# jakubbober/discrete-curvature-rewiring

Hardware: AMD Instinct MI355X
Metric: SDRF iterations/sec (higher is better)
Workload: dtype f64; 1 GPU; S100k: preferential-attachment graph N=100000 m=10 E=999900 (PCG64 seed 12345), Balanced Forman curvature, full recompute every iteration, remove_edges=True, tau=163.0, removal_bound=0.95; parallelism=single GPU

## Files before the change

### discrete-curvature-rewiring_amd/csrc/dcr_bfc_h2.hip

```cpp
#include <algorithm>
#include <climits>
#include <cstdio>
#include <cstdlib>
#include <cstring>
#include <vector>

#include "dcr_bfc_common.h"

namespace dcr {

constexpr unsigned H2_EMPTY = 0xFFFFFFFFu;
constexpr unsigned H2_NBR = 0x80000000u;
constexpr int H2_CLASSES = 5;
constexpr int H2_WB = 4;
__device__ inline unsigned h2_rec_t(int T, int deg) { return (unsigned)T | ((unsigned)deg << 16); }
static_assert(H2_MAXDEG < 65536, "record packing");
constexpr int H2_SMALL_DEG = 64;
#ifndef H2_Q
#define H2_Q 2
#endif
#ifndef H2_QL
#define H2_QL 2
#endif
constexpr int H2_QCAP = 128;
// ... 993 lines not shown
    int pln = sc->pln;
#pragma unroll 1
    while (true) {
        const int i = lcur + lane;
        const unsigned item = i < ls.n ? ls.items[i] : 0xFFFFFFFFu;
        const bool mine = i < ls.n && (int)(item >> 19) == bidx;
        const int cnt = __popcll(__ballot(mine));
        if (cnt == 0) break;
        const int s = (int)(item & 0x1FFFu), r = (int)((item >> 13) & 63u);
        const unsigned w = mine ? t.key[s] : 0u;
        h2_settle<L1, EXS>(t, sc, mine, mine ? s : -1, r, w, pln, tk, al, tbase);
        lcur += cnt;
        if (cnt < 64) break;
    }
    if (lane == 0) sc->pln = pln;
    h2_wave_sync();
}

__device__ inline void h2_batch_begin(const H2Tasks tk, H2Alloc &al, H2Scratch *sc, int k, int &tbase, int &trow, int rev = -1) {
    const int lane = threadIdx.x & 63;
    const unsigned long long below = (1ull << lane) - 1ull;
    sc->rowT[lane] = 0;
    sc->rowPos[lane] = 0;
    sc->rowMx[lane] = 0;
    sc->rowRev[lane] = rev;
    if (lane == 0) sc->pln = 0;
    int dummy_c, dummy_p;
    const unsigned long long rows = __ballot(k >= 0);
    if (!h2_pool_reserve(tk, al, __popcll(rows), 0, 0, tbase, dummy_c, dummy_p)) tbase = -1;
    trow = __popcll(rows & below);
    sc->trank[lane] = (unsigned char)trow;
    trow += tbase;
}

template <int L1, int EXS, bool PARTS>
__device__ inline void h2_batch_end(const View &g, const H2Tasks tk, H2Alloc &al, int u, int2 ru, int i, int k, int2 rk, int tbase,
                                    int trow, int part, const H2Tab t, H2Scratch *sc, uint4 *rec, const unsigned *items = nullptr,
                                    int ifrom = 0, int ito = 0) {
    const int lane = threadIdx.x & 63;
    int T = sc->rowT[lane], pos = sc->rowPos[lane], mx = sc->rowMx[lane];
    const int rev = sc->rowRev[lane];
    bool listed = tbase >= 0 && k >= 0 && T > 0 && pos > 0 && rev >= 0 && rev < g.cap_total;
    int ep;
    const int Pn = h2_prefix(listed ? T : 0, ep);
    int p0 = 0;
    if (Pn > 0) {
        int dummy_t, dummy_c;
        if (!h2_pool_reserve(tk, al, 0, 0, Pn, dummy_t, dummy_c, p0)) listed = false;
    }
    if (__ballot(listed) != 0ull) {
        const int pln = sc->pln;
        if (pln <= H2_PLCAP) {
            sc->poff[lane] = listed ? p0 + ep : -1;
            h2_wave_sync();
            for (int j = lane; j < pln; j += 64) {
                const int r = sc->plr[j];
                if (sc->poff[r] >= 0) tk.part[atomicAdd(&sc->poff[r], 1)] = (int32_t)sc->plt[j];
            }
            h2_wave_sync();
        } else if (items) {
            sc->poff[lane] = listed ? p0 + ep : -1;
            h2_wave_sync();
            for (int j = ifrom + lane; j < ito; j += 64) {
                const unsigned item = items[j];
                const int s2 = (int)(item & 0x1FFFu), r = (int)((item >> 13) & 63u);
                if ((h2_cnt_get(t.cnt, s2) & 0x8000u) && sc->poff[r] >= 0) tk.part[atomicAdd(&sc->poff[r], 1)] = (int32_t)t.key[s2];
            }
            h2_wave_sync();
        } else {
            const bool shortrow = listed && rk.y <= H2_SHORT_ROW;
            if (shortrow) h2_partners_short<L1, EXS>(g, tk, u, rk, p0 + ep, T, t);
            unsigned long long todo = __ballot(listed && !shortrow);
            while (todo) {
                const int l = __ffsll((long long)todo) - 1;
                todo &= todo - 1;
                const int2 rv = make_int2(__shfl(rk.x, l), __shfl(rk.y, l));
                h2_partners_of_row<L1, EXS>(g, tk, u, rv, __shfl(p0 + ep, l), __shfl(T, l), t);
            }
        }
    }
    if (tbase >= 0 && k >= 0) {
        tk.task[trow] = listed ? make_uint4((unsigned)(ru.x + i), (unsigned)(p0 + ep), (unsigned)T, (unsigned)u | tk.retry_flag)
                               : make_uint4(0u, 0u, H2_TASK_VOID, 0u);
    }
    if (listed) {
        pos = 0;
        mx = 0;
    }
    if (k >= 0) {
        const int64_t slot = (int64_t)ru.x + i;
        if (rev < 0 || rev >= g.cap_total) {
            row_ok(g, make_int2(-1, rev), 33, u, k);
        } else if (!PARTS) {
            rec[slot] = make_uint4((unsigned)pos, (unsigned)mx, h2_rec_t(T, ru.y), (unsigned)rev);
        } else {
            unsigned *r4 = reinterpret_cast<unsigned *>(rec + slot);
            if (pos) atomicAdd(&r4[0], (unsigned)pos);
            if (mx) atomicMax(&r4[1], (unsigned)mx);
            if (part == 0) {
                r4[2] = h2_rec_t(T, ru.y);
                r4[3] = (unsigned)rev;
            }
        }
    }
}

constexpr int H2_JOIN_MAXM = 256;
__device__ inline int h2_probe_partners(const H2EdgeSet es, int w, const int32_t *pt, int np);

template <int L1, int EXS, int NW>
__device__ inline bool h2_join_prepare(const View &g, const H2Tab t, int2 ru, const H2List &ls) {
    constexpr int NT = 64 * NW, PER = EXS / NT;
    static_assert(PER >= 2 && PER % 2 == 0, "a thread owns whole cursor words");
    static_assert(EXS / 2 <= (1 << L1) / 32, "the cursors fit B1");
    static_assert(NW * H2_ITEMS < 65536 && EXS <= 8192, "16-bit cursors, 13-bit slots");
    const int tid = (int)threadIdx.x, lane = tid & 63, wid = tid >> 6;
    unsigned *cur = t.b1;
    int n[PER], sum = 0, most = 0;
#pragma unroll
    for (int q = 0; q < PER; ++q) {
        const unsigned c16 = h2_cnt_get(t.cnt, tid * PER + q);
        n[q] = ((c16 & 0x8000u) || c16 < 2u) ? 0 : (int)c16;
        sum += n[q];
        most = n[q] > most ? n[q] : most;
    }
    if (__syncthreads_or(most > H2_JOIN_MAXM)) return false;
    int excl;
    const int wtot = h2_prefix(sum, excl);
    if (lane == 0) t.wsum[wid] = wtot;
    __syncthreads();
    int off = excl;
    for (int w = 0; w < wid; ++w) off += t.wsum[w];
#pragma unroll
    for (int q = 0; q < PER; q += 2) {
        const unsigned lo = (unsigned)off;
        off += n[q];
        const unsigned hi = (unsigned)off;
        off += n[q + 1];
        cur[(tid * PER + q) >> 1] = lo | (hi << 16);
    }
    __syncthreads();
    for (int base = 0; base < ls.n; base += 64) {
        const int j = base + lane;
        if (j >= ls.n) continue;
        const unsigned item = ls.items[j];
        const int s = (int)(item & 0x1FFFu), r = (int)((item >> 13) & 63u), b = (int)(item >> 19);
        const unsigned c16 = h2_cnt_get(t.cnt, s);
        if ((c16 & 0x8000u) || c16 < 2u) continue;
        const int row = (b * 64 + r) * NW + wid;
        if (row >= ru.y) {
            row_ok(g, make_int2(-1, row), 44, ru.y, (int)item);
            continue;
        }
        const int v = g.col[ru.x + row];
        const unsigned old = atomicAdd(&cur[s >> 1], 1u << ((s & 1) * 16));
        const int p = (int)((old >> ((s & 1) * 16)) & 0xFFFFu);
        if (p < NW * H2_ITEMS) ls.srt[p] = v;
        else row_ok(g, make_int2(-1, p), 45, s, (int)c16);
    }
    __syncthreads();
    return true;
}

template <int L1, int EXS, int NW, bool PARTS>
__device__ inline void h2_batch_join(const View &g, const H2Tasks tk, H2Alloc &al, int u, int2 ru, int i, int k, int2 rk, int part,
                                     const H2Tab t, H2Scratch *sc, uint4 *rec, const H2List &ls, int &lcur, int bidx, int rev) {
    const int lane = threadIdx.x & 63;
    sc->rowT[lane] = 0;
    sc->rowPos[lane] = 0;
    sc->rowMx[lane] = 0;
    sc->rowRev[lane] = rev;
    if (lane == 0) sc->pln = 0;
    h2_wave_sync();
    const int lfrom = lcur;
#pragma unroll 1
    while (true) {
        const int j = lcur + lane;
        const unsigned item = j < ls.n ? ls.items[j] : 0xFFFFFFFFu;
        const bool mine = j < ls.n && (int)(item >> 19) == bidx;
        const int cnt = __popcll(__ballot(mine));
        if (cnt == 0) break;
        if (mine && (h2_cnt_get(t.cnt, (int)(item & 0x1FFFu)) & 0x8000u)) atomicAdd(&sc->rowT[(item >> 13) & 63u], 1);
        lcur += cnt;
        if (cnt < 64) break;
    }
    h2_wave_sync();
    const unsigned *cur = t.b1;
#pragma unroll 1
    for (int base = lfrom; base < lcur; base += 64) {
        const int j = base + lane;
        const bool have = j < lcur;
        const unsigned item = have ? ls.items[j] : 0u;
        const int s = (int)(item & 0x1FFFu), r = (int)((item >> 13) & 63u);
        const int vr = __shfl(k, r);
        if (!have) continue;
        const unsigned c16 = h2_cnt_get(t.cnt, s);
        if (c16 & 0x8000u) continue;
        const int m = (int)(c16 & 0x7FFFu);
        int c = m - 1;
        if (c <= 0) continue;
        if (sc->rowT[r] > 0 && vr >= 0) {
            const int end = (int)((cur[s >> 1] >> ((s & 1) * 16)) & 0xFFFFu);
            if (end >= m && end <= NW * H2_ITEMS) {
                c -= h2_probe_partners(tk.es, vr, ls.srt + (end - m), m);
            } else {
                row_ok(g, make_int2(-1, end), 46, s, m);
                c = 0;
            }
        }
        if (c > 0) {
            atomicAdd(&sc->rowPos[r], 1);
            atomicMax(&sc->rowMx[r], c);
        }
    }
    h2_wave_sync();
    h2_batch_end<L1, EXS, PARTS>(g, tk, al, u, ru, i, k, rk, -1, 0, part, t, sc, rec);
}

template <int L1, int EXS, int NW, bool PARTS, int PHASE>
__device__ inline void h2_stream(const View &g, const H2Tasks tk, H2Alloc &al, int u, int2 ru, int part, int nparts,
                                 const H2Tab t, H2Scratch *sc, uint4 *rec, int k0, int2 rk0, H2List &ls) {
    const int lane = threadIdx.x & 63;
    const int wid = (int)(threadIdx.x >> 6);
    int qn = 0;
    int lcur = 0;
    if (PHASE == 0 && ru.y > 64 * NW * H2_REV_BATCHES) ls.over = true;
    for (int base = 0; base < ru.y; base += 64 * NW) {
        const int i = base + lane * NW + wid;
        int k = k0;
        int2 rk = rk0;
        if (base > 0) {
            k = -1;
            rk = make_int2(0, 0);
            if (i < ru.y) {
                k = g.col[ru.x + i];
                if (k >= 0 && k < g.n && k != u) {
                    rk = g.rowinfo[k];
                    if (!row_ok(g, rk, 32, k, u)) rk = make_int2(0, 0);
                } else {
                    k = -1;
                }
            }
        }
        const int np = rk.y > 0 ? ((rk.x + rk.y + 3) >> 2) - (rk.x >> 2) : 0;
        int poff_lane;
        const int P = h2_prefix(np, poff_lane);
        if (P == 0) continue;
        const int bidx = base / (64 * NW);
        int tbase = -1, trow = 0;
        if (PHASE == 2 && !ls.over) {
            if (ls.join) {
                h2_batch_join<L1, EXS, NW, PARTS>(g, tk, al, u, ru, i, k, rk, part, t, sc, rec, ls, lcur, bidx, ls.revs[bidx * 64 + lane]);
                h2_wave_sync();
                continue;
            }
            h2_batch_begin(tk, al, sc, k, tbase, trow, ls.revs[bidx * 64 + lane]);
            h2_wave_sync();
            const int lfrom = lcur;
            h2_settle_items<L1, EXS>(t, sc, ls, lcur, bidx, tk, al, tbase);
            h2_batch_end<L1, EXS, PARTS>(g, tk, al, u, ru, i, k, rk, tbase, trow, part, t, sc, rec, ls.items, lfrom, lcur);
            h2_wave_sync();
            continue;
        }
        if (PHASE == 0 && !ls.over) ls.revs[bidx * 64 + lane] = -1;
        sc->desc[lane] = rk;
        sc->poff[lane] = poff_lane;
        if (lane == 0) sc->poff[64] = P;
        if (PHASE == 2) h2_batch_begin(tk, al, sc, k, tbase, trow);
        h2_wave_sync();
        const bool listing = PHASE == 1 && !ls.over;
        auto flags = [&](const int4 w, unsigned vm, int r, int a) -> unsigned {
            const unsigned kk[4] = {(unsigned)w.x, (unsigned)w.y, (unsigned)w.z, (unsigned)w.w};
            const unsigned isu = h2_eq4(kk, (unsigned)u) & vm;
            if (PHASE == 2 && isu) sc->rowRev[r] = a + __ffs((int)isu) - 1;
            if (listing && isu) ls.revs[bidx * 64 + r] = a + __ffs((int)isu) - 1;
            unsigned valid = vm & ~isu;
            if (PARTS && PHASE != 2 && !listing) {
#pragma unroll
                for (int jj = 0; jj < 4; ++jj)
                    if (h2_part(kk[jj], nparts) != part) valid &= ~(1u << jj);
            }
            if (PHASE == 0) {
                h2_mark4<L1>(t.b1, t.b2, kk, valid);
                return 0u;
            }
            return h2_again4<L1>(t.b2, kk, valid);
        };
        h2_for_pieces_queued<(PARTS ? H2_QL : H2_Q)>(g.col, sc->desc, sc->poff, poff_lane, P, qn, flags,
                             [&](int idx, unsigned key, int r) {
                                 sc->qw[idx] = key;
                                 if (PHASE != 0) sc->qr[idx] = (unsigned char)r;
                                 if (PHASE == 1) sc->qb[idx] = (unsigned char)bidx;
                             },
                             [&]() { h2_drain<L1, EXS, PHASE, PARTS>(t, sc, qn, tk, al, tbase, ls, part, nparts); });
        if (PHASE == 2) {
            h2_drain<L1, EXS, PHASE, PARTS>(t, sc, qn, tk, al, tbase, ls, part, nparts);
            h2_batch_end<L1, EXS, PARTS>(g, tk, al, u, ru, i, k, rk, tbase, trow, part, t, sc, rec);
        }
        h2_wave_sync();
    }
    if (qn > 0) h2_drain<L1, EXS, PHASE, PARTS>(t, sc, qn, tk, al, -1, ls, part, nparts);
}

constexpr int H2_NPB = 12;
template <int L1, int EXS, int NW, bool PARTS>
__device__ inline bool h2_node_fast(const View &g, const H2Tasks tk, H2Alloc &al, int u, int2 ru, int part, int nparts,
                                    const H2Tab t, H2Scratch *sc, uint4 *rec, bool &ok, H2List &ls) {
    const int tid = (int)threadIdx.x, lane = tid & 63, wid = tid >> 6;
    constexpr int NT = 64 * NW, NP = H2_NPB;
    const unsigned long long below = (1ull << lane) - 1ull;
    if (ru.y > 64 * NW) return false;
    const int i = lane * NW + wid;
    int k = -1;
    int2 rk = make_int2(0, 0);
    if (i < ru.y) {
        k = g.col[ru.x + i];
        if (k >= 0 && k < g.n && k != u) {
            rk = g.rowinfo[k];
            if (!row_ok(g, rk, 32, k, u)) rk = make_int2(0, 0);
        } else {
            k = -1;
        }
    }
    const int np = rk.y > 0 ? ((rk.x + rk.y + 3) >> 2) - (rk.x >> 2) : 0;
    int poff_lane;
    const int P = h2_prefix(np, poff_lane);
    if (__syncthreads_or(P > 64 * NP)) return false;
    {
        uint4 *z = reinterpret_cast<uint4 *>(t.b1);
        constexpr int NZ = ((1 << L1) / 32 + (1 << (L1 - 2)) / 32) / 4;
        for (int j = tid; j < NZ; j += NT) z[j] = make_uint4(0u, 0u, 0u, 0u);
        uint4 *k4 = reinterpret_cast<uint4 *>(t.key);
        for (int j = tid; j < EXS / 4; j += NT) k4[j] = make_uint4(H2_EMPTY, H2_EMPTY, H2_EMPTY, H2_EMPTY);
        uint4 *c4 = reinterpret_cast<uint4 *>(t.cnt);
        for (int j = tid; j < EXS / 8; j += NT) c4[j] = make_uint4(0u, 0u, 0u, 0u);
        if (tid == 0) *t.full = 0;
    }
    sc->desc[lane] = rk;
    sc->poff[lane] = poff_lane;
    if (lane == 0) sc->poff[64] = P;
    h2_wave_sync();
    int4 w[NP];
    unsigned long long meta[NP];
#pragma unroll
    for (int q = 0; q < NP; ++q) {
        const int j = 64 * q + lane;
        w[q] = make_int4(0, 0, 0, 0);
        meta[q] = 0ull;
        const int jf = 64 * q, jl = jf + 63 < P ? jf + 63 : P - 1;
        if (jf >= P) continue;
        const int r = h2_piece_row(sc->poff, poff_lane, j < P ? j : jl, jf, jl);
        if (j < P) {
            const int2 d = sc->desc[r];
            const int a = (d.x & ~3) + 4 * (j - sc->poff[r]);
            w[q] = load_piece(g.col, a);
            meta[q] = (unsigned long long)h2_piece_mask(a, d.x, d.x + d.y) | ((unsigned long long)r << 8) | ((unsigned long long)(unsigned)a << 16);
        }
    }
    __syncthreads();
    if (k >= 0) {
        const int sl = h2_insert<EXS>(t.key, (unsigned)k);
        if (sl < 0) *t.full = 1;
        else h2_cnt_flag(t.cnt, sl);
        h2_seed<L1>(t.b1, t.b2, (unsigned)k);
    }
    __syncthreads();
#pragma unroll
    for (int q = 0; q < NP; ++q) {
        if (64 * q >= P) continue;
        const unsigned kk[4] = {(unsigned)w[q].x, (unsigned)w[q].y, (unsigned)w[q].z, (unsigned)w[q].w};
        unsigned valid = (unsigned)meta[q] & 0xFu & ~h2_eq4(kk, (unsigned)u);
        if (PARTS) {
#pragma unroll
            for (int jj = 0; jj < 4; ++jj)
                if (h2_part(kk[jj], nparts) != part) valid &= ~(1u << jj);
        }
        meta[q] |= (unsigned long long)valid << 4;
        h2_mark4<L1>(t.b1, t.b2, kk, valid);
    }
    __syncthreads();
    int qn = 0, tbase = -1, trow = 0;
    sc->rowRev[lane] = -1;
    h2_wave_sync();
    {
        unsigned fl[NP];
#pragma unroll
        for (int q = 0; q < NP; ++q) {
            fl[q] = 0u;
            if (64 * q >= P) continue;
            const unsigned kk[4] = {(unsigned)w[q].x, (unsigned)w[q].y, (unsigned)w[q].z, (unsigned)w[q].w};
            const unsigned valid = (unsigned)(meta[q] >> 4) & 0xFu;
            const unsigned isu = h2_eq4(kk, (unsigned)u) & (unsigned)meta[q] & 0xFu;
            if (isu) sc->rowRev[(int)((meta[q] >> 8) & 0xFFull)] = (int)(meta[q] >> 16) + __ffs((int)isu) - 1;
            fl[q] = h2_again4<L1>(t.b2, kk, valid);
        }
#pragma unroll 1
        while (true) {
            bool stop = false;
#pragma unroll
            for (int q = 0; q < NP; ++q) {
                if (64 * q >= P) continue;
                const unsigned kk[4] = {(unsigned)w[q].x, (unsigned)w[q].y, (unsigned)w[q].z, (unsigned)w[q].w};
#pragma unroll
                for (int jj = 0; jj < 4; ++jj) {
                    const bool p = (fl[q] >> jj) & 1u;
                    const unsigned long long m = __ballot(p);
                    if (m == 0ull) continue;
                    if (stop || qn + __popcll(m) > H2_QCAP) {
                        stop = true;
                        continue;
                    }
                    if (p) {
                        const int idx = qn + __popcll(m & below);
                        sc->qw[idx] = kk[jj];
                        sc->qr[idx] = (unsigned char)((meta[q] >> 8) & 0xFFull);
                        sc->qb[idx] = 0;
                        fl[q] &= ~(1u << jj);
                    }
                    qn += __popcll(m);
                }
            }
            if (qn > 0) h2_drain<L1, EXS, 1, PARTS>(t, sc, qn, tk, al, -1, ls, part, nparts);
            if (!stop) break;
        }
    }
    __syncthreads();
    ok = *t.full == 0;
    ls.join = !__syncthreads_or(ls.over) && ok;
    if (ls.join) ls.join = h2_join_prepare<L1, EXS, NW>(g, t, ru, ls);
    if (ls.join) {
        int lcur = 0;
        const int myrev = sc->rowRev[lane];
        h2_wave_sync();
        h2_batch_join<L1, EXS, NW, PARTS>(g, tk, al, u, ru, i, k, rk, part, t, sc, rec, ls, lcur, 0, myrev);
    } else if (ok) {
        if (tid == 0) atomicAdd(&tk.res->h2_fallback, 1);
        if (!ls.over) {
            int lcur = 0;
            const int myrev = sc->rowRev[lane];
            h2_wave_sync();
            h2_batch_begin(tk, al, sc, k, tbase, trow, myrev);
            h2_wave_sync();
            h2_settle_items<L1, EXS>(t, sc, ls, lcur, 0, tk, al, tbase);
            h2_batch_end<L1, EXS, PARTS>(g, tk, al, u, ru, i, k, rk, tbase, trow, part, t, sc, rec, ls.items, 0, lcur);
        } else {
            h2_stream<L1, EXS, NW, PARTS, 2>(g, tk, al, u, ru, part, nparts, t, sc, rec, k, rk, ls);
        }
    }
    __syncthreads();
    return true;
}

template <int L1, int EXS, int NW, bool PARTS>
__device__ inline bool h2_node(const View &g, const H2Tasks tk, H2Alloc &al, int u, int2 ru, int part, int nparts,
                               const H2Tab t, H2Scratch *sc, uint4 *rec, H2List &ls) {
    const int tid = (int)threadIdx.x;
    constexpr int NT = 64 * NW;
    if constexpr (!PARTS) {
        bool ok_fast = true;
        if (h2_node_fast<L1, EXS, NW, PARTS>(g, tk, al, u, ru, part, nparts, t, sc, rec, ok_fast, ls)) return ok_fast;
    }
    int k0 = -1;
    int2 rk0 = make_int2(0, 0);
    {
        const int i0 = (tid & 63) * NW + (tid >> 6);
        if (i0 < ru.y) {
            k0 = g.col[ru.x + i0];
            if (k0 >= 0 && k0 < g.n && k0 != u) {
                rk0 = g.rowinfo[k0];
                if (!row_ok(g, rk0, 32, k0, u)) rk0 = make_int2(0, 0);
            } else {
                k0 = -1;
            }
        }
    }
    {
        uint4 *z = reinterpret_cast<uint4 *>(t.b1);
        constexpr int NZ = ((1 << L1) / 32 + (1 << (L1 - 2)) / 32) / 4;
        for (int i = tid; i < NZ; i += NT) z[i] = make_uint4(0u, 0u, 0u, 0u);
        uint4 *k4 = reinterpret_cast<uint4 *>(t.key);
        for (int i = tid; i < EXS / 4; i += NT) k4[i] = make_uint4(H2_EMPTY, H2_EMPTY, H2_EMPTY, H2_EMPTY);
        uint4 *c4 = reinterpret_cast<uint4 *>(t.cnt);
        for (int i = tid; i < EXS / 8; i += NT) c4[i] = make_uint4(0u, 0u, 0u, 0u);
        if (tid == 0) *t.full = 0;
    }
    __syncthreads();
    for (int i = tid; i < ru.y; i += NT) {
        const int k = g.col[ru.x + i];
        if (k >= 0 && k < g.n && k != u) {
            const int s = h2_insert<EXS>(t.key, (unsigned)k);
            if (s < 0) *t.full = 1;
            else h2_cnt_flag(t.cnt, s);
            h2_seed<L1>(t.b1, t.b2, (unsigned)k);
        }
    }
    __syncthreads();
    h2_stream<L1, EXS, NW, PARTS, 0>(g, tk, al, u, ru, part, nparts, t, sc, rec, k0, rk0, ls);
    __syncthreads();
    h2_stream<L1, EXS, NW, PARTS, 1>(g, tk, al, u, ru, part, nparts, t, sc, rec, k0, rk0, ls);
    __syncthreads();
    const bool ok = *t.full == 0;
    ls.join = !__syncthreads_or(ls.over) && ok;
    if (ls.join) ls.join = h2_join_prepare<L1, EXS, NW>(g, t, ru, ls);
    if (!ls.join && ok && tid == 0) atomicAdd(&tk.res->h2_fallback, 1);
    if (ok) h2_stream<L1, EXS, NW, PARTS, 2>(g, tk, al, u, ru, part, nparts, t, sc, rec, k0, rk0, ls);
    __syncthreads();
    return ok;
}

template <int L1, int EXS, int NW, bool PARTS>
__global__ void __launch_bounds__(64 * NW) __attribute__((amdgpu_waves_per_eu(3))) k_h2_block(View g, H2Tasks tk, const int4 *units, const int32_t *count, int64_t unit_cap,
                                                       uint4 *rec, H2Retry rt, int is_retry) {
    __shared__ __attribute__((aligned(16))) unsigned bits[(1 << L1) / 32 + (1 << (L1 - 2)) / 32];
    __shared__ __attribute__((aligned(16))) unsigned key[EXS];
    __shared__ __attribute__((aligned(16))) unsigned cnt[EXS / 2];
    __shared__ H2Scratch sc_all[NW];
    __shared__ int full;
    __shared__ int wsum[NW];
    const int wid = threadIdx.x >> 6;
    const int total = *count;
    if (total < 0 || total > unit_cap) {
        row_ok(g, make_int2(-1, total), 37, 0, 0);
        return;
    }
    const H2Tab t{bits, bits + (1 << L1) / 32, key, cnt, &full, wsum};
    H2Alloc al;
    for (int64_t it = blockIdx.x; it < total; it += gridDim.x) {
        const int4 un = units[it];
        const int u = un.x;
        const int nparts = PARTS ? (int)((unsigned)un.y >> 16) : 1, part = PARTS ? (un.y & 0xFFFF) : 0;
        bool ok = u >= 0 && u < g.n && nparts >= 1 && part < nparts;
        int2 ru = make_int2(0, 0);
        if (ok) {
            ru = g.rowinfo[u];
            ok = row_ok(g, ru, 38, u, (int)it) && ru.y > 0 && ru.y <= H2_MAXDEG;
        }
        if (!ok) continue;
        H2List ls = h2_list_of(tk.lists, NW);
        const bool unit_ok = h2_node<L1, EXS, NW, PARTS>(g, tk, al, u, ru, part, nparts, t, &sc_all[wid], rec, ls);
        if (!unit_ok) {
            if (threadIdx.x == 0) {
                if (is_retry) {
                    rt.res->h2_status = 1;
                    atomicAdd(&rt.res->h2_failed[5], 1);
                } else {
                    h2_retry_push(rt, u, ru.y, PARTS ? 4 : 3);
                }
            }
        }
    }
    h2_void_candidates(tk, al.c_cur, al.c_end);
    h2_void_tasks(tk, al.t_cur, al.t_end);
}

__device__ inline int h2_probe_partners(const H2EdgeSet es, int w, const int32_t *pt, int np) {
    int found = 0;
    for (int j = 0; j < np; j += 8) {
        int tt[8];
#pragma unroll
        for (int q = 0; q < 8; ++q) tt[q] = j + q < np ? pt[j + q] : -1;
        unsigned long long key[8], k0[8], h[8];
        unsigned bw[8], bb[8];
#pragma unroll
        for (int q = 0; q < 8; ++q) {
            key[q] = h2_edge_key(w, tt[q] < 0 ? w : tt[q]);
            bb[q] = h2_bloom_bit(key[q], es.bloom_bits);
            bw[q] = es.bloom[bb[q] >> 5];
        }
#pragma unroll
        for (int q = 0; q < 8; ++q) {
            const bool maybe = tt[q] >= 0 && ((bw[q] >> (bb[q] & 31u)) & 1u);
            h[q] = h2_eset_slot(key[q], es.bits);
            k0[q] = maybe ? es.tab[h[q]] : H2_ESET_EMPTY;
        }
#pragma unroll
        for (int q = 0; q < 8; ++q) {
            bool hit = k0[q] == key[q];
            if (!hit && k0[q] != H2_ESET_EMPTY) hit = h2_eset_has(es, w, tt[q]);
            found += hit ? 1 : 0;
        }
    }
    return found;
}

__global__ void __launch_bounds__(256) k_h2_triangles(H2EdgeSet es, H2Tasks tk, uint4 *rec, const int32_t *status, int second) {
    const int cand_now = *tk.n_cand;
    const int first = second ? *tk.n_done : 0;
    const int total = cand_now < tk.cand_cap ? cand_now : (int)tk.cand_cap;
    if (!second && blockIdx.x == 0 && threadIdx.x == 0) *tk.n_done = cand_now;
    if (*status != 0) return;
    if (total <= first || first < 0) return;
    const int lane = threadIdx.x & 63;
    for (int64_t base = first + (((int64_t)blockIdx.x * 256 + threadIdx.x) & ~63ll); base < total; base += (int64_t)gridDim.x * 256) {
        const int64_t i = base + lane;
        int c = 0;
        unsigned slot = 0xFFFFFFFFu;
        if (i < total) {
            const int4 cd = tk.cand[i];
            const uint4 ts = (cd.z >= 0 && cd.z < tk.task_cap) ? tk.task[cd.z] : make_uint4(0u, 0u, H2_TASK_VOID, 0u);
            const bool skip = ts.z == H2_TASK_VOID || (!(ts.w & 0x80000000u) && ((unsigned)tk.weight[ts.w & 0x7FFFFFFFu] & 0x80000000u));
            if (!skip) {
                slot = ts.x;
                c = cd.y - h2_probe_partners(es, cd.x, tk.part + ts.y, (int)ts.z);
            }
        }
        const unsigned prev = (unsigned)__shfl_up((int)slot, 1);
        const bool head = lane == 0 || prev != slot;
        const unsigned long long heads = __ballot(head);
        const int seg = __popcll(heads & ((2ull << lane) - 1ull));
        int n = c > 0 ? 1 : 0, mx = c > 0 ? c : 0;
#pragma unroll
        for (int off = 1; off < 64; off <<= 1) {
            const int s2 = __shfl_up(seg, off), n2 = __shfl_up(n, off), m2 = __shfl_up(mx, off);
            if (lane >= off && s2 == seg) {
                n += n2;
                mx = m2 > mx ? m2 : mx;
            }
        }
        const bool tail = lane == 63 || ((heads >> (lane + 1)) & 1ull);
        if (tail && n > 0 && slot != 0xFFFFFFFFu) {
            unsigned *r4 = reinterpret_cast<unsigned *>(rec + slot);
            atomicAdd(&r4[0], (unsigned)n);
            atomicMax(&r4[1], (unsigned)mx);
        }
    }
}

__global__ void __launch_bounds__(256) k_h2_weight(View g, int32_t *weight) {
    const int64_t s = (int64_t)blockIdx.x * 256 + threadIdx.x;
    const int lane = threadIdx.x & 63;
    int u = -1, val = 0;
    if (s < g.cap_total) {
        const int us = g.slot_row[s];
        const int v = g.col[s];
        const bool uok = us >= 0 && us < g.n, vok = v >= 0 && v < g.n;
        const int2 ru = g.rowinfo[uok ? us : 0];
        const int dv = g.rowinfo[vok ? v : 0].y;
        if (uok) {
            u = us;
            if (vok && s >= ru.x && (int)(s - ru.x) < ru.y) val = dv;
        }
    }
#pragma unroll
    for (int off = 1; off < 64; off <<= 1) {
        const int t = __shfl_up(val, off), uu = __shfl_up(u, off);
        if (lane >= off && uu == u) val += t;
    }
    const int un = __shfl_down(u, 1);
    if (u >= 0 && val > 0 && (lane == 63 || un != u)) atomicAdd(&weight[u], val);
}

constexpr int H2_NB = H2_CLASSES * H2_WB;
__device__ inline void h2_clear_result(DevResult *res, int tid, int half, bool flags_cleared) {
    if (tid == 0 && flags_cleared) res->touched_n = 0;
    if (tid < 8) res->misc[tid] = 0;
    if (tid < H2_NB) {
        res->h2_bucket[half][tid] = 0;
        res->h2_fill[half][tid] = 0;
    }
    if (tid < H2_CLASSES) res->h2_count[tid] = 0;
    if (tid == 0) {
        res->h2_status = 0;
        res->h2_retry = 0;
        for (int p = 0; p < 2; ++p) res->h2_ntask[p] = res->h2_ncand[p] = res->h2_npart[p] = res->h2_ncand_done[p] = 0;
        for (int c = 0; c < 6; ++c) res->h2_failed[c] = 0;
        res->h2_fallback = 0;
        res->flag_too_big = 0;
    }
}
struct H2Lists {
    int4 *units[H2_CLASSES];
    int64_t cap[H2_CLASSES];
};
constexpr int H2_PLAN_THREADS = 1024;

__device__ inline void h2_classify(int d, int S, int &cls, int &wb, int &nparts) {
    nparts = 1;
    int lo = 0;
    if (d <= H2_SMALL_DEG && S <= h2_maxw(2)) {
        cls = S <= h2_maxw(0) ? 0 : S <= h2_maxw(1) ? 1 : 2;
        lo = cls == 0 ? 0 : h2_maxw(cls - 1);
        wb = (int)((int64_t)(S - lo) * H2_WB / (h2_maxw(cls) - lo + 1));
    } else if (S <= h2_maxw(3) && d + S / 4 <= h2_keycap(3)) {
// ... 158 lines not shown
        bool want[Q];
#pragma unroll
        for (int q = 0; q < Q; ++q) {
            const int64_t s = s0 + q * stride;
            const bool in = s < g.cap_total;
            u[q] = in ? g.slot_row[s] : -1;
            v[q] = in ? g.col[s] : -1;
            a[q] = in ? rec[s] : make_uint4(0u, 0u, 0u, 0u);
        }
        int2 ru[Q];
        int dv[Q], rcol[Q], rrow[Q];
        uint4 b[Q];
        bool rok[Q];
#pragma unroll
        for (int q = 0; q < Q; ++q) {
            want[q] = u[q] >= 0 && u[q] < g.n && v[q] > u[q] && v[q] < g.n;
            const int64_t r = (int64_t)a[q].w;
            rok[q] = want[q] && r >= 0 && r < g.cap_total;
            ru[q] = make_int2(0, 0);
            dv[q] = 0;
            rcol[q] = rrow[q] = -1;
            b[q] = make_uint4(0u, 0u, 0u, 0u);
            if (want[q]) ru[q] = g.rowinfo[u[q]];
            if (rok[q]) {
                b[q] = rec[r];
                dv[q] = (int)(b[q].z >> 16);
                if (s0 + q * stride == 0) {
                    rcol[q] = g.col[r];
                    rrow[q] = g.slot_row[r];
                } else {
                    rcol[q] = (int64_t)b[q].w == s0 + q * stride ? u[q] : -1;
                    rrow[q] = v[q];
                }
            }
        }
#pragma unroll
        for (int q = 0; q < Q; ++q) {
            const int64_t s = s0 + q * stride;
            if (!want[q]) continue;
            if (s < ru[q].x || (int)(s - ru[q].x) >= ru[q].y) continue;
            double val;
            if (ru[q].y == 1 || (rok[q] && dv[q] == 1)) {
                val = 0.0;
            } else {
                if (!rok[q] || rcol[q] != u[q] || rrow[q] != v[q]) {
                    row_ok(g, make_int2(-1, (int)a[q].w), 39, u[q], v[q]);
                    continue;
                }
                if ((a[q].z & 0xFFFFu) != (b[q].z & 0xFFFFu) || (int)(a[q].z >> 16) != ru[q].y) {
                    row_ok(g, make_int2(-1, (int)a[q].z), 40, u[q], v[q]);
                    continue;
                }
                const int gam = (int)(a[q].y > b[q].y ? a[q].y : b[q].y);
                val = bfc_formula(ru[q].y, dv[q], (int)(a[q].z & 0xFFFFu), (int)b[q].x, (int)a[q].x, gam);
            }
            curv[s] = val;
            ext_take(lo_v, lo_s, val, (int)s, 0);
            ext_take(hi_v, hi_s, val, (int)s, 1);
        }
    }
    ext_wave_reduce(lo_v, lo_s, 0);
    ext_wave_reduce(hi_v, hi_s, 1);
    if ((threadIdx.x & 63) == 0) {
        const int w = (int)blockIdx.x * 4 + (int)(threadIdx.x >> 6);
        part_min[w] = ext_make(lo_v, lo_s);
        part_max[w] = ext_make(hi_v, hi_s);
    }
}

bool h2_grow_pools(dcr_graph *g) {
    const DevResult &h = *g->hres.p;
    const int64_t t = std::max(h.h2_ntask[0], h.h2_ntask[1]), c = std::max(h.h2_ncand[0], h.h2_ncand[1]), p = std::max(h.h2_npart[0], h.h2_npart[1]);
    if (h.h2_ntask[0] < 0 || h.h2_ntask[1] < 0 || h.h2_ncand[0] < 0 || h.h2_ncand[1] < 0 || h.h2_npart[0] < 0 || h.h2_npart[1] < 0) return false;
    if (t < 0 || c < 0 || p < 0) return false;
    g->h2_want[0] = std::max<int64_t>(g->h2_want[0], 2 * t + 4096);
    g->h2_want[1] = std::max<int64_t>(g->h2_want[1], 2 * c + 65536);
    g->h2_want[2] = std::max<int64_t>(g->h2_want[2], 2 * p + 65536);
    return true;
}

static int ensure_h2(dcr_graph *g) {
    if (g->h2_weight.cap < g->n + 64) g->h2_weight_valid = false;
    DCR_TRY(g->h2_weight.grow(g->n + 64));
    DCR_TRY(g->h2_rec.grow(g->cap_total + 64));
    int bits = 10;
    while ((1ll << bits) < g->cap_total) ++bits;
    if (g->h2_eset_bits != bits || !g->h2_eset.p) {
        DCR_TRY(g->h2_eset.alloc((int64_t)1 << bits));
        g->h2_eset_bits = bits;
        g->h2_eset_valid = false;
    }
    int bbits = 16;
    while ((1ll << bbits) < 4 * g->cap_total) ++bbits;
    if (g->h2_bloom_bits != bbits || !g->h2_bloom.p) {
        DCR_TRY(g->h2_bloom.alloc(((int64_t)1 << bbits) / 32));
        g->h2_bloom_bits = bbits;
        g->h2_eset_valid = false;
    }
    const int64_t need[H2_CLASSES] = {g->n + 64, g->n + 64, g->n + 64, g->n + 64, g->n + g->cap_total / 4 + 64};
    for (int c = 0; c < H2_CLASSES; ++c) DCR_TRY(g->h2_units[c].grow(need[c]));
    DCR_TRY(g->h2_retry.grow(g->n + g->cap_total / 4 + 64));
    DCR_TRY(g->h2_task.grow(2 * std::max<int64_t>(g->cap_total + 4096, g->h2_want[0])));
    DCR_TRY(g->h2_cand.grow(2 * std::max<int64_t>(2 * g->cap_total + 65536, g->h2_want[1])));
    DCR_TRY(g->h2_part.grow(2 * std::max<int64_t>(g->cap_total + 65536, g->h2_want[2])));
    const int cus = g->num_cu > 0 ? g->num_cu : 256;
    DCR_TRY(g->h2_lists.grow((int64_t)cus * (16 + 12) * H2_LIST_WORDS));
    return DCR_OK;
}

template <int C>
static void launch_h2_small(dcr_graph *g, const View &vw, const H2Retry &rt, hipStream_t st) {
    constexpr int H2_WPB = h2_wpb(C);
    constexpr int NP = h2_maxw(C) / 256 + 1;
    auto kern = k_h2_small<h2_l1(C), h2_exs(C), h2_clcap(C), H2_WPB, NP>;
    static int per_cu_res = 0;
    if (per_cu_res == 0) {
        int nb = 0;
        if (hipOccupancyMaxActiveBlocksPerMultiprocessor(&nb, kern, 64 * H2_WPB, 0) != hipSuccess || nb < 1) {
            (void)hipGetLastError();
            nb = (160 * 1024) / (H2_WPB * (int)sizeof(H2Small<h2_l1(C), h2_exs(C), h2_clcap(C)>));
            if (nb > 32 / H2_WPB) nb = 32 / H2_WPB;
        }
        per_cu_res = nb < 1 ? 1 : nb;
    }
    int64_t grid = (int64_t)g->num_cu * per_cu_res;
    const int64_t units = g->h2_last_count[C] >= 0 ? (int64_t)g->h2_last_count[C] + g->h2_last_count[C] / 32 + 8 : g->n;
    if (grid > (units + H2_WPB - 1) / H2_WPB) grid = (units + H2_WPB - 1) / H2_WPB;
    if (grid < 1) grid = 1;
    hipLaunchKernelGGL(kern, dim3((unsigned)grid), dim3(64 * H2_WPB), 0, st, vw,
                       g->h2_units[C].p, &g->dres.p->h2_count[C], g->h2_units[C].cap, g->h2_rec.p, rt);
}

template <int C, bool PARTS>
static void launch_h2_block(dcr_graph *g, const View &vw, const H2Tasks &tk, const H2Retry &rt, const int4 *units,
                            const int32_t *count, int64_t cap, int64_t units_hint, int is_retry, hipStream_t st) {
    int64_t grid = units_hint;
    const int64_t most = (int64_t)g->num_cu * (C == 3 ? 3 : 1);
    if (grid > most) grid = most;
    if (grid < 1) grid = 1;
    hipLaunchKernelGGL((k_h2_block<h2_l1(C), h2_exs(C), h2_waves(C), PARTS>), dim3((unsigned)grid), dim3(64 * h2_waves(C)), 0,
                       st, vw, tk, units, count, cap, g->h2_rec.p, rt, is_retry);
}

int launch_curvature_pass_h2(dcr_graph *g) {
    if (g->num_cu <= 0) {
        g->num_cu = 256;
        hipDeviceProp_t prop;
        if (hipGetDeviceProperties(&prop, g->device) == hipSuccess && prop.multiProcessorCount > 0)
            g->num_cu = prop.multiProcessorCount;
    }
    DCR_TRY(ensure_h2(g));
    View vw{g->rowinfo.p, g->col.p, g->slot_row.p, g->cap_total, g->dres.p->misc, nullptr, (int32_t)g->n, 0};
    H2Lists L;
    for (int c = 0; c < H2_CLASSES; ++c) {
        L.units[c] = g->h2_units[c].p;
        L.cap[c] = g->h2_units[c].cap;
    }
    int32_t *status = &g->dres.p->h2_status;
    const H2Retry rt{g->h2_retry.p, g->h2_retry.cap, g->h2_weight.p, g->dres.p};
    const int64_t tcap = g->h2_task.cap / 2, ccap = g->h2_cand.cap / 2, pcap = g->h2_part.cap / 2;
    DevResult *dr = g->dres.p;
    unsigned *lists_L = g->h2_lists.p, *lists_M = g->h2_lists.p + (int64_t)g->num_cu * 16 * H2_LIST_WORDS;
    const H2EdgeSet es{g->h2_eset.p, g->h2_eset_bits, g->h2_bloom.p, g->h2_bloom_bits};
    H2Tasks tk{g->h2_task.p, g->h2_cand.p, g->h2_part.p, tcap, ccap, pcap, &dr->h2_ntask[0], &dr->h2_ncand[0], &dr->h2_npart[0],
               &dr->h2_ncand_done[0], g->dres.p, g->h2_weight.p, 0u, lists_L, es};
    const H2Tasks tkM{g->h2_task.p + tcap, g->h2_cand.p + ccap, g->h2_part.p + pcap, tcap, ccap, pcap, &dr->h2_ntask[1], &dr->h2_ncand[1],
                      &dr->h2_npart[1], &dr->h2_ncand_done[1], g->dres.p, g->h2_weight.p, 0u, lists_M, es};
    const int64_t sblocks = (g->cap_total + 255) / 256;
    const int64_t pblocks = (g->n + H2_PLAN_THREADS - 1) / H2_PLAN_THREADS;
    const bool whole = g->n % 4 == 0;
    unsigned *dirty_words = reinterpret_cast<unsigned *>(g->dirty.p);
    const int64_t n_dirty_words = whole ? g->n / 4 : (int64_t)0;
    const bool run_weight = !g->h2_weight_valid;
    const bool fast_head = !run_weight && g->h2_head_clean && pblocks > 0;
    const int parity = g->h2_parity & 1;
    g->h2_head_clean = false;
    if (!fast_head) {
        const int64_t cb = (g->n + 255) / 256;
        hipLaunchKernelGGL(k_h2_clear, dim3((unsigned)(cb < 1 ? 1 : cb > 2048 ? 2048 : cb)), dim3(256), 0, g->stream, g->dres.p, g->h2_weight.p,
                           run_weight ? g->n : (int64_t)0, dirty_words, n_dirty_words);
        if (run_weight && sblocks > 0) hipLaunchKernelGGL(k_h2_weight, dim3((unsigned)sblocks), dim3(256), 0, g->stream, vw, g->h2_weight.p);
        g->h2_weight_valid = true;
    }
    g->h2_cleared_dirty = whole;
    const bool patch = pblocks > 0 && g->h2_eset_valid && g->h2_eset_pending <= EDIT_LOG_CAP &&
                       g->h2_eset_tombs + g->h2_eset_pending <= ((int64_t)1 << g->h2_eset_bits) / 16;
    const bool journal = patch && g->h2_eset_pending > 0;
    if (pblocks > 0) {
        hipLaunchKernelGGL(k_h2_plan<0>, dim3((unsigned)pblocks), dim3(H2_PLAN_THREADS), 0, g->stream, vw, g->h2_weight.p, L,
                           g->dres.p, parity, fast_head ? 1 : 0, dirty_words, n_dirty_words, g->h2_rec.p, es, 0);
        hipLaunchKernelGGL(k_h2_plan<1>, dim3((unsigned)(pblocks + (journal ? 1 : 0))), dim3(H2_PLAN_THREADS), 0, g->stream, vw,
                           g->h2_weight.p, L, g->dres.p, parity, fast_head ? 1 : 0, dirty_words, n_dirty_words, g->h2_rec.p, es, journal ? 1 : 0);
    }
    if (!fast_head)
        hipLaunchKernelGGL(k_h2_retry_zero, dim3(1024), dim3(256), 0, g->stream, vw, g->h2_units[4].p, &g->dres.p->h2_count[4], g->h2_units[4].cap,
                           g->h2_rec.p);
    g->h2_parity = 1 - parity;
    g->h2_weight_launches += run_weight ? 1 : 0;
    g->h2_clear_launches += fast_head ? 0 : 1;
    static const int three_streams[H2_CLASSES] = {0, 1, 2, 0, 2}, five_streams[H2_CLASSES] = {0, 1, 2, 3, 4};
    const int *lay = g->n < 400000 ? three_streams : five_streams;
    hipStream_t pool[5] = {g->stream, g->side[1], g->low[0], g->low[1], g->side[2]};
    hipEvent_t done[5] = {nullptr, g->ev_join[1], g->ev_join[2], g->ev_join[3], g->ev_aux2};
    bool used[5] = {true, false, false, false, false};
    DCR_HIP(hipEventRecord(g->ev_fork, g->stream));
    auto on = [&](int c) {
        const int si = lay[c];
        if (!used[si]) {
            used[si] = true;
            (void)hipStreamWaitEvent(pool[si], g->ev_fork, 0);
        }
        return pool[si];
    };
    bool eset_on_aux = false;
    if (patch) {
        if (journal) g->h2_eset_tombs += g->h2_eset_pending;
    } else {
        DCR_HIP(hipStreamWaitEvent(g->aux, g->ev_fork, 0));
        DCR_HIP(hipMemsetAsync(g->h2_eset.p, 0xFF, sizeof(unsigned long long) << g->h2_eset_bits, g->aux));
        DCR_HIP(hipMemsetAsync(g->h2_bloom.p, 0, sizeof(unsigned) * (((size_t)1 << g->h2_bloom_bits) / 32), g->aux));
        if (sblocks > 0) hipLaunchKernelGGL(k_h2_eset_build, dim3((unsigned)sblocks), dim3(256), 0, g->aux, vw, es, status, g->dres.p);
        g->h2_eset_tombs = 0;
        DCR_HIP(hipEventRecord(g->ev_aux, g->aux));
        eset_on_aux = true;
    }
    g->h2_eset_valid = true;
    g->h2_eset_pending = 0;
    const int64_t hint4 = g->h2_last_count[4] >= 0 ? (int64_t)g->h2_last_count[4] + 8 : g->num_cu;
    const int64_t hint3 = g->h2_last_count[3] >= 0 ? (int64_t)g->h2_last_count[3] + 8 : 3 * (int64_t)g->num_cu;
    hipStream_t st_split = on(0), st_mid = on(1);
    if (eset_on_aux) {
        DCR_HIP(hipStreamWaitEvent(st_split, g->ev_aux, 0));
        if (st_mid != st_split) DCR_HIP(hipStreamWaitEvent(st_mid, g->ev_aux, 0));
    }
    launch_h2_block<4, true>(g, vw, tk, rt, g->h2_units[4].p, &g->dres.p->h2_count[4], g->h2_units[4].cap, hint4, 0, st_split);
    launch_h2_block<3, false>(g, vw, tkM, rt, g->h2_units[3].p, &g->dres.p->h2_count[3], g->h2_units[3].cap, hint3, 0, st_mid);
    const bool tri_stage = g->h2_expect_triangles;
    if (tri_stage) {
        hipLaunchKernelGGL(k_h2_triangles, dim3((unsigned)(g->num_cu * 4)), dim3(256), 0, pool[lay[0]], es, tk, g->h2_rec.p, status, 0);
        hipLaunchKernelGGL(k_h2_triangles, dim3((unsigned)(g->num_cu * 8)), dim3(256), 0, pool[lay[1]], es, tkM, g->h2_rec.p, status, 0);
    }
    launch_h2_small<2>(g, vw, rt, on(2));
    launch_h2_small<1>(g, vw, rt, on(3));
    launch_h2_small<0>(g, vw, rt, on(4));
    for (int si = 1; si < 5; ++si)
        if (used[si]) {
            DCR_HIP(hipEventRecord(done[si], pool[si]));
            DCR_HIP(hipStreamWaitEvent(g->stream, done[si], 0));
        }
    if (!g->ext_part.p) DCR_TRY(g->ext_part.alloc(2 * EXT_PART_BLOCKS));
    int64_t fblocks = (sblocks + H2_FINAL_Q - 1) / H2_FINAL_Q;
    if (fblocks > H2_FINAL_BLOCKS) fblocks = H2_FINAL_BLOCKS;
    if (fblocks > EXT_PART_BLOCKS / 4) fblocks = EXT_PART_BLOCKS / 4;
    if (fblocks < 1) fblocks = 1;
    const bool retry_stage = g->h2_expect_retry;
    if (retry_stage) {
        hipLaunchKernelGGL(k_h2_retry_zero, dim3(1024), dim3(256), 0, g->stream, vw, g->h2_retry.p, &g->dres.p->h2_retry, g->h2_retry.cap,
                           g->h2_rec.p);
        tk.retry_flag = 0x80000000u;
        launch_h2_block<4, true>(g, vw, tk, rt, g->h2_retry.p, &g->dres.p->h2_retry, g->h2_retry.cap, 64, 1, g->stream);
        if (tri_stage)
            hipLaunchKernelGGL(k_h2_triangles, dim3((unsigned)(g->num_cu * 2)), dim3(256), 0, g->stream, es, tk, g->h2_rec.p, status, 1);
    }
    hipLaunchKernelGGL(k_h2_final, dim3((unsigned)fblocks), dim3(256), 0, g->stream, vw, g->h2_rec.p, g->curv.p, status, g->ext_part.p,
                       g->ext_part.p + EXT_PART_BLOCKS, &g->dres.p->h2_retry, retry_stage ? 1 : 0, &g->dres.p->h2_fallback,
                       tri_stage ? 1 : 0);
    g->h2_launches += 1;
    g->h2_last_retry_stage = retry_stage;
    g->h2_last_tri_stage = tri_stage;
    g->ext_part_n = (int)fblocks * 4;
    g->ext_part_valid = true;
    DCR_HIP(hipGetLastError());
    g->h2_head_clean = pblocks > 0;
    return DCR_OK;
}

__global__ void __launch_bounds__(256) k_h2_weight_diff(const int32_t *kept, const int32_t *fresh, int64_t n, int32_t *out) {
    int bad = 0;
    for (int64_t i = (int64_t)blockIdx.x * 256 + threadIdx.x; i < n; i += (int64_t)gridDim.x * 256)
        bad += (kept[i] & 0x7FFFFFFF) != fresh[i];
    if (bad) atomicAdd(out, bad);
}

int h2_weight_check(dcr_graph *g, int64_t *mismatches) {
    *mismatches = -1;
    if (!g->h2_weight_valid || !g->h2_weight.p) return DCR_OK;
    DCR_TRY(g->h2_weight_chk.grow(g->n + 64));
    int32_t *fresh = g->h2_weight_chk.p, *count = g->h2_weight_chk.p + g->n;
    DCR_HIP(hipMemsetAsync(fresh, 0, sizeof(int32_t) * (size_t)(g->n + 1), g->stream));
    View vw{g->rowinfo.p, g->col.p, g->slot_row.p, g->cap_total, g->dres.p->misc, nullptr, (int32_t)g->n, 0};
    const int64_t sblocks = (g->cap_total + 255) / 256, cb = (g->n + 255) / 256;
    if (sblocks > 0) hipLaunchKernelGGL(k_h2_weight, dim3((unsigned)sblocks), dim3(256), 0, g->stream, vw, fresh);
    hipLaunchKernelGGL(k_h2_weight_diff, dim3((unsigned)(cb < 1 ? 1 : cb > 2048 ? 2048 : cb)), dim3(256), 0, g->stream, g->h2_weight.p, fresh,
                       g->n, count);
    DCR_HIP(hipGetLastError());
    int32_t bad = 0;
    DCR_HIP(hipMemcpyAsync(&bad, count, sizeof(int32_t), hipMemcpyDeviceToHost, g->stream));
    DCR_HIP(hipStreamSynchronize(g->stream));
    *mismatches = bad;
    return DCR_OK;
}

}
```

Baseline: 1226 iterations/sec.

## Add row-bitmask path for small-degree nodes in H2 curvature kernel

Adds a specialized path for nodes with degree up to 128 that records, for each 2-hop candidate, a 128-bit mask of which neighbour rows reach it, plus per-row adjacency masks. Square/4-cycle counts then come from popcounts of mask differences instead of the queued per-row drain and batch logic. If the tables overflow, the path clears them and falls back to the original flow, which can duplicate work. It also adds a global atomic counter of row-path successes and failures, with a host query function.

```diff
diff --git a/discrete-curvature-rewiring_amd/csrc/dcr_bfc_h2.hip b/discrete-curvature-rewiring_amd/csrc/dcr_bfc_h2.hip
--- a/discrete-curvature-rewiring_amd/csrc/dcr_bfc_h2.hip
+++ b/discrete-curvature-rewiring_amd/csrc/dcr_bfc_h2.hip
@@ -1319,14 +1319,151 @@
     if (qn > 0) h2_drain<L1, EXS, PHASE, PARTS>(t, sc, qn, tk, al, -1, ls, part, nparts);
 }
 
+constexpr int H2_ROWS_MAX = 128;
+constexpr int H2_ROWS_EXS = 1024;
+constexpr int H2_ROWS_CL = 2048;
+__device__ unsigned h2_rows_units[2];
+
+__device__ inline int h2r_find_or_insert(unsigned *exkey, unsigned w) {
+    unsigned s = h2s_home<H2_ROWS_EXS>(w);
+#pragma unroll 1
+    for (int walk = 0; walk < H2_WALK; ++walk) {
+        const unsigned e = exkey[s];
+        if ((e & ~H2_NBR) == w && e != H2_EMPTY) return (int)s;
+        if (e == H2_EMPTY) {
+            const unsigned old = atomicCAS(&exkey[s], H2_EMPTY, w);
+            if (old == H2_EMPTY || (old & ~H2_NBR) == w) return (int)s;
+        }
+        s = (s + 1) & (unsigned)(H2_ROWS_EXS - 1);
+    }
+    return -1;
+}
+
+template <int L1, int EXS, int NW, int NP>
+__device__ inline bool h2_rows_unit(const View &g, int u, int2 ru, int i, int k, int P, const int4 (&w)[NP], unsigned long long (&meta)[NP],
+                                    const H2Tab t, H2Scratch *sc, uint4 *rec) {
+    static_assert(EXS >= 4 * H2_ROWS_EXS, "the row masks fit the counting table's keys");
+    static_assert(EXS / 2 >= H2_ROWS_EXS + 6 * H2_ROWS_MAX, "the exact keys, adjacency masks and row results fit its counts");
+    static_assert((1 << L1) / 32 >= H2_ROWS_CL, "the candidate list fits B1");
+    static_assert(64 * NW >= H2_ROWS_MAX && H2_ROWS_MAX <= 256 && H2_ROWS_EXS <= 65536, "a row per lane; 8-bit rows, 16-bit slots");
+    const int tid = (int)threadIdx.x, lane = tid & 63, wid = tid >> 6;
+    constexpr int NT = 64 * NW;
+    const unsigned long long below = (1ull << lane) - 1ull;
+    unsigned *exm = t.key;
+    unsigned *exkey = t.cnt;
+    unsigned *adj = t.cnt + H2_ROWS_EXS;
+    int *pos = reinterpret_cast<int *>(adj + 4 * H2_ROWS_MAX), *mx = pos + H2_ROWS_MAX;
+    unsigned *cl = t.b1;
+    int *cln = t.wsum;
+    bool full = *t.full != 0;
+    int qn = 0;
+    auto drain = [&]() {
+        h2_wave_sync();
+        for (int base = 0; base < qn; base += 64) {
+            const int j = base + lane;
+            bool cand = false;
+            int slot = -1, row = 0;
+            if (j < qn) {
+                row = sc->qr[j];
+                slot = h2r_find_or_insert(exkey, sc->qw[j]);
+                if (slot < 0) {
+                    full = true;
+                } else if (row >= ru.y) {
+                    row_ok(g, make_int2(-1, row), 47, u, ru.y);
+                } else if (exkey[slot] & H2_NBR) {
+                    const unsigned x = exm[4 * slot];
+                    if (x >= (unsigned)ru.y) row_ok(g, make_int2(-1, (int)x), 48, u, ru.y);
+                    else atomicOr(&adj[4 * row + (int)(x >> 5)], 1u << (x & 31u));
+                } else {
+                    atomicOr(&exm[4 * slot + (row >> 5)], 1u << (row & 31));
+                    cand = true;
+                }
+            }
+            const unsigned long long m = __ballot(cand);
+            if (m == 0ull) continue;
+            int first = 0;
+            if (lane == 0) first = atomicAdd(cln, __popcll(m));
+            first = __shfl(first, 0);
+            if (cand) {
+                const int idx = first + __popcll(m & below);
+                if (idx < H2_ROWS_CL) cl[idx] = (unsigned)slot | ((unsigned)row << 16);
+                else full = true;
+            }
+        }
+        h2_wave_sync();
+        qn = 0;
+    };
+    {
+        constexpr int FL = 48;
+        int nfl = 0;
+#pragma unroll
+        for (int q = 0; q < NP; ++q) {
+            if (64 * q >= P) continue;
+            const unsigned kk[4] = {(unsigned)w[q].x, (unsigned)w[q].y, (unsigned)w[q].z, (unsigned)w[q].w};
+            const unsigned isu = h2_eq4(kk, (unsigned)u) & (unsigned)meta[q] & 0xFu;
+            if (isu) sc->rowRev[(int)((meta[q] >> 8) & 0xFFull)] = (int)(meta[q] >> 16) + __ffs((int)isu) - 1;
+            const unsigned f = h2_again4<L1>(t.b2, kk, (unsigned)(meta[q] >> 4) & 0xFu);
+            meta[q] |= (unsigned long long)f << FL;
+            nfl += __popc(f);
+        }
+        int qi;
+        const int qtotal = h2_prefix_dpp(nfl, qi);
+#pragma unroll 1
+        for (int left = qtotal; left > 0; left -= H2_QCAP) {
+#pragma unroll
+            for (int q = 0; q < NP; ++q) {
+                if (64 * q >= P) continue;
+                while ((meta[q] >> FL) != 0ull && qi < H2_QCAP) {
+                    const unsigned f = (unsigned)(meta[q] >> FL), b = f & (0u - f);
+                    sc->qw[qi] = h2_pick4(w[q], b);
+                    sc->qr[qi] = (unsigned char)((int)((meta[q] >> 8) & 0xFFull) * NW + wid);
+                    meta[q] ^= (unsigned long long)b << FL;
+                    ++qi;
+                }
+            }
+            qn = left < H2_QCAP ? left : H2_QCAP;
+            drain();
+            if (__ballot(full) != 0ull) break;
+            qi -= H2_QCAP;
+        }
+    }
+    if (__syncthreads_or(full)) return false;
+    const int cl_n = *cln;
+    const uint4 *exm4 = reinterpret_cast<const uint4 *>(exm), *adj4 = reinterpret_cast<const uint4 *>(adj);
+    for (int e = tid; e < cl_n; e += NT) {
+        const unsigned item = cl[e];
+        const int row = (int)(item >> 16);
+        const uint4 m = exm4[item & 0xFFFFu], a = adj4[row];
+        const int c = __popc(m.x & ~a.x) + __popc(m.y & ~a.y) + __popc(m.z & ~a.z) + __popc(m.w & ~a.w) - 1;
+        if (c > 0) {
+            atomicAdd(&pos[row], 1);
+            atomicMax(&mx[row], c);
+        }
+    }
+    __syncthreads();
+    if (k >= 0) {
+        const int rev = sc->rowRev[lane];
+        if (rev < 0 || rev >= g.cap_total) {
+            row_ok(g, make_int2(-1, rev), 33, u, k);
+        } else {
+            const uint4 a = adj4[i];
+            const int T = __popc(a.x) + __popc(a.y) + __popc(a.z) + __popc(a.w);
+            rec[(int64_t)ru.x + i] = make_uint4((unsigned)pos[i], (unsigned)mx[i], h2_rec_t(T, ru.y), (unsigned)rev);
+        }
+    }
+    return true;
+}
+
 constexpr int H2_NPB = 12;
 template <int L1, int EXS, int NW, bool PARTS>
 __device__ inline bool h2_node_fast(const View &g, const H2Tasks tk, H2Alloc &al, int u, int2 ru, int part, int nparts,
                                     const H2Tab t, H2Scratch *sc, uint4 *rec, bool &ok, H2List &ls) {
     const int tid = (int)threadIdx.x, lane = tid & 63, wid = tid >> 6;
     constexpr int NT = 64 * NW, NP = H2_NPB;
+    constexpr bool ROWS = !PARTS && NW == 4 && EXS >= 4 * H2_ROWS_EXS;
     const unsigned long long below = (1ull << lane) - 1ull;
     if (ru.y > 64 * NW) return false;
+    const bool rows = ROWS && ru.y <= H2_ROWS_MAX;
     const int i = lane * NW + wid;
     int k = -1;
     int2 rk = make_int2(0, 0);
@@ -1343,16 +1480,21 @@
     int poff_lane;
     const int P = h2_prefix(np, poff_lane);
     if (__syncthreads_or(P > 64 * NP)) return false;
-    {
+    auto clear = [&](bool for_rows) {
+        const uint4 zero = make_uint4(0u, 0u, 0u, 0u), none = make_uint4(H2_EMPTY, H2_EMPTY, H2_EMPTY, H2_EMPTY);
         uint4 *z = reinterpret_cast<uint4 *>(t.b1);
         constexpr int NZ = ((1 << L1) / 32 + (1 << (L1 - 2)) / 32) / 4;
-        for (int j = tid; j < NZ; j += NT) z[j] = make_uint4(0u, 0u, 0u, 0u);
+        for (int j = tid; j < NZ; j += NT) z[j] = zero;
         uint4 *k4 = reinterpret_cast<uint4 *>(t.key);
-        for (int j = tid; j < EXS / 4; j += NT) k4[j] = make_uint4(H2_EMPTY, H2_EMPTY, H2_EMPTY, H2_EMPTY);
+        for (int j = tid; j < EXS / 4; j += NT) k4[j] = for_rows ? zero : none;
         uint4 *c4 = reinterpret_cast<uint4 *>(t.cnt);
-        for (int j = tid; j < EXS / 8; j += NT) c4[j] = make_uint4(0u, 0u, 0u, 0u);
-        if (tid == 0) *t.full = 0;
-    }
+        for (int j = tid; j < EXS / 8; j += NT) c4[j] = (for_rows && j < H2_ROWS_EXS / 4) ? none : zero;
+        if (tid == 0) {
+            *t.full = 0;
+            t.wsum[0] = 0;
+        }
+    };
+    clear(rows);
     sc->desc[lane] = rk;
     sc->poff[lane] = poff_lane;
     if (lane == 0) sc->poff[64] = P;
@@ -1375,12 +1517,22 @@
         }
     }
     __syncthreads();
-    if (k >= 0) {
+    auto seed_table = [&]() {
         const int sl = h2_insert<EXS>(t.key, (unsigned)k);
         if (sl < 0) *t.full = 1;
         else h2_cnt_flag(t.cnt, sl);
+    };
+    if (k >= 0) {
+        if (rows) {
+            const int sl = h2s_insert_nbr<H2_ROWS_EXS>(t.cnt, (unsigned)k);
+            if (sl < 0) *t.full = 1;
+            else t.key[4 * sl] = (unsigned)i;
+        } else {
+            seed_table();
+        }
         h2_seed<L1>(t.b1, t.b2, (unsigned)k);
     }
+    if (rows) sc->rowRev[lane] = -1;
     __syncthreads();
 #pragma unroll
     for (int q = 0; q < NP; ++q) {
@@ -1396,6 +1548,27 @@
         h2_mark4<L1>(t.b1, t.b2, kk, valid);
     }
     __syncthreads();
+    if constexpr (ROWS) {
+        if (rows) {
+            const bool done = h2_rows_unit<L1, EXS, NW, NP>(g, u, ru, i, k, P, w, meta, t, sc, rec);
+            if (tid == 0) atomicAdd(&h2_rows_units[done ? 0 : 1], 1u);
+            __syncthreads();
+            if (done) {
+                ok = true;
+                return true;
+            }
+            {
+                uint4 *k4 = reinterpret_cast<uint4 *>(t.key);
+                for (int j = tid; j < EXS / 4; j += NT) k4[j] = make_uint4(H2_EMPTY, H2_EMPTY, H2_EMPTY, H2_EMPTY);
+                uint4 *c4 = reinterpret_cast<uint4 *>(t.cnt);
+                for (int j = tid; j < EXS / 8; j += NT) c4[j] = make_uint4(0u, 0u, 0u, 0u);
+                if (tid == 0) *t.full = 0;
+            }
+            __syncthreads();
+            if (k >= 0) seed_table();
+            __syncthreads();
+        }
+    }
     int qn = 0, tbase = -1, trow = 0;
     sc->rowRev[lane] = -1;
     h2_wave_sync();
@@ -2160,3 +2333,9 @@
 }
 
 }
+
+extern "C" int dcr_h2_rowmask_units(uint32_t out[2]) {
+    const unsigned zero[2] = {0u, 0u};
+    if (!out || hipMemcpyFromSymbol(out, HIP_SYMBOL(dcr::h2_rows_units), sizeof zero) != hipSuccess) return DCR_EHIP;
+    return hipMemcpyToSymbol(HIP_SYMBOL(dcr::h2_rows_units), zero, sizeof zero) == hipSuccess ? DCR_OK : DCR_EHIP;
+}
```

New measurement: 1255 iterations/sec (median of 6 runs). 1.02x the previous value.
